# Simple-Robotics/proxsuite

Measured on AMD Instinct MI355X. Metric: QPs/sec (batch, dense backend) at fixed (n, n_eq, n_in); max |KKT residual| vs ref, higher is better.
Workload: dtype f64; 1 GPU; c2: 2048 random dense fp64 QPs per GPU, n=100 n_eq=50 n_in=100, eps_abs=1e-09 eps_rel=0 NO_INITIAL_GUESS (reference generators and seeds, benchmark/timings-parallel.cpp:43-63; BASELINE.json configs); batch_per_gpu=2048, n=100, n_eq=50, n_in=100, threads_per_qp=64, lds_bytes_per_qp=18968, parallelism=batch sharded over 1 GPU(s), dense_backend=PrimalDualLDLT

## Files before the change

### proxsuite_amd/csrc/pqp_capi.hip

```cpp
#include <hip/hip_runtime.h>

#include <algorithm>
#include <cmath>
#include <cstdio>
#include <cstdlib>
#include <cstring>
#include <limits>
#include <string>
#include <vector>

#include "pqp_host.hpp"
#include "pqp_diag.hpp"

namespace {

thread_local std::string g_err;

bool
absent(double v)
{
  return std::isnan(v);
}

int
// ... 254 lines not shown
  const int need = d.nd > d.n ? d.nd : d.n;
  h->nt = need <= 256 ? 256 : (need <= 512 ? 512 : 1024);
  if (need > PQP_MAX_ROWS || pqp::setup_lds_bytes(d, 1024) > 160 * 1024) {
    delete h;
    return fail(PQP_ERR_UNSUPPORTED, "max(n, n_eq + n_in (+ n)) > " + std::to_string(PQP_MAX_ROWS) +
                                       " (or n + n_eq + n_in (+ n) > ~10000) is not supported by this build");
  }
#if PQP_CHUNK_ALL
  if (const char* e = std::getenv("PQP_TEST_NT_MAX")) {
    const int f = std::atoi(e);
    if ((f == 256 || f == 512) && h->nt > f)
      h->nt = f;
  }
#endif
  if (const char* e = std::getenv("PQP_SCHEDULE"))
    h->lpt = std::string(e) == "lpt";
  h->dev.rep_phase = 0;
  h->dev.rep_count = 1;
  h->dev.trace = nullptr;
  h->dev.trace_slot = nullptr;
  h->dev.trace_cap = 0;
  if (const char* e = std::getenv("PQP_REPEAT_PHASE"))
    h->dev.rep_phase = std::atoi(e);
  if (const char* e = std::getenv("PQP_REPEAT_COUNT"))
    h->dev.rep_count = std::atoi(e);
  h->lds_solve = pqp::lds_bytes(d, h->nt);
  h->lds_setup = pqp::setup_lds_bytes(d, h->nt);
  const char* force_hbm = std::getenv("PQP_FORCE_HBM_VECTORS");
  const bool vectors_in_hbm = h->lds_solve > 160 * 1024 || (force_hbm && force_hbm[0] == '1');
  if (vectors_in_hbm)
    h->nt = 1024;
  const size_t B = size_t(batch_size), n = size_t(dim), ne = size_t(n_eq), ni = size_t(n_in),
               nc = size_t(d.nc), nd = size_t(d.nd);
  pqp::Batch& D = h->dev;
  int rc = 0;
#define ALLOC(ptr, cnt)                                                                             \
  if ((rc = dalloc(h, &(ptr), (cnt)))) {                                                            \
    pqp_batch_destroy(h);                                                                           \
    return rc;                                                                                      \
  }                                                                                                 \
  if (B > 0 && size_t(cnt) % B == 0 && (void*)(ptr) != (void*)h->d_order && (void*)(ptr) != (void*)h->d_cmd)           \
    h->per_qp.push_back({ reinterpret_cast<char*>(ptr), (size_t(cnt) / B) * sizeof(*(ptr)) });
  ALLOC(D.H, B * n * n)
  ALLOC(D.g, B * n)
  ALLOC(D.A, B * ne * n)
  ALLOC(D.b, B * ne)
  ALLOC(D.C, B * ni * n)
  ALLOC(D.u, B * ni)
  ALLOC(D.l, B * ni)
  ALLOC(D.u_box, B * n)
  ALLOC(D.l_box, B * n)
  ALLOC(D.Hs, B * n * n)
  ALLOC(D.gs, B * n)
  ALLOC(D.As, B * ne * n)
  ALLOC(D.ATs, B * ne * n)
  ALLOC(D.bs, B * ne)
  ALLOC(D.Cs, B * ni * n)
  ALLOC(D.CTs, B * ni * n)
  ALLOC(D.us, B * ni)
  ALLOC(D.ls, B * ni)
  ALLOC(D.ubs, B * n)
  ALLOC(D.lbs, B * n)
  ALLOC(D.is, B * n)
  ALLOC(D.delta, B * size_t(d.ntot))
  ALLOC(D.x, B * n)
  ALLOC(D.y, B * ne)
  ALLOC(D.z, B * nc)
  ALLOC(D.se, B * ne)
  ALLOC(D.si, B * nc)
  ALLOC(D.info, B)
  ALLOC(D.state, B)
  ALLOC(D.F, B * n * n)
  ALLOC(D.WL, B * n * n)
  ALLOC(D.WU, B * n * n)
  ALLOC(D.dF, B * n)
  ALLOC(D.Zr, B * nd * n)
  ALLOC(D.Zc, B * nd * n)
  ALLOC(D.G, B * nd * nd)
  ALLOC(D.WS, B * nd * nd)
  ALLOC(D.LS, B * nd * nd)
  ALLOC(D.dS, B * nd)
  ALLOC(D.act, B * nc)
  ALLOC(D.stats, B * size_t(pqp::ST_COUNT))
  if (vectors_in_hbm) {
    h->lds_solve = pqp::lds_bytes(d, h->nt);
    h->lds_setup = pqp::setup_lds_bytes(d, h->nt);
    if ((rc = dalloc(h, &h->vec_scratch, B * ((h->lds_solve + 7) / 8)))) {
      pqp_batch_destroy(h);
      return rc;
    }
  }
  ALLOC(h->d_order, B)
  ALLOC(h->d_settings, B)
  ALLOC(h->d_cmd, B)
#undef ALLOC
  D.settings = h->d_settings;
  D.cmd = h->d_cmd;

  h->settings.resize(B);
  for (auto& s : h->settings)
    pqp_settings_default(&s, h->backend);
  h->cmd.assign(B, pqp::Cmd{});
  h->is_initialized.assign(B, 0);
  h->c_diag.assign(B, 0);
  {
    std::vector<pqp_info> info(B);
    for (auto& i : info)
      pqp_info_default(&i, h->backend);
    if (B)
      HIP_TRY(hipMemcpy(D.info, info.data(), B * sizeof(pqp_info), hipMemcpyHostToDevice));
    std::vector<pqp::State> st(B);
    for (auto& s : st) {
      std::memset(&s, 0, sizeof(s));
      s.ruiz_c = 1.0;
    }
    if (B)
      HIP_TRY(hipMemcpy(D.state, st.data(), B * sizeof(pqp::State), hipMemcpyHostToDevice));
    const double ib = std::sqrt(std::numeric_limits<double>::max());
    std::vector<double> tmp;
    auto fill = [&](double* dst, size_t cnt, double v) -> int {
      if (!cnt)
        return PQP_OK;
      tmp.assign(cnt, v);
      HIP_TRY(hipMemcpy(dst, tmp.data(), cnt * sizeof(double), hipMemcpyHostToDevice));
      return PQP_OK;
    };
    if ((rc = fill(D.u, B * ni, +ib)) || (rc = fill(D.l, B * ni, -ib)) ||
        (rc = fill(D.u_box, B * n, +ib)) || (rc = fill(D.l_box, B * n, -ib)) ||
        (rc = fill(D.delta, B * size_t(d.ntot), 1.0)) || (rc = fill(D.is, B * n, 1.0))) {
      pqp_batch_destroy(h);
      return rc;
    }
  }
  HIP_TRY(hipEventCreate(&h->ev0));
  HIP_TRY(hipEventCreate(&h->ev1));
  HIP_TRY(hipEventCreate(&h->ev_mid));
  *out = h;
  return PQP_OK;
}

void
pqp_batch_destroy(pqp_batch* h)
{
  if (!h)
    return;
  (void)settle(h);
  DeviceGuard guard_(h->device);
  for (void* p : h->host_allocs)
    (void)hipHostFree(p);
  if (h->owned_stream)
    (void)hipStreamDestroy(h->owned_stream);
  for (void* p : h->allocs)
    (void)hipFree(p);
  if (h->trace_dev)
    (void)hipFree(h->trace_dev);
  if (h->trace_slot_dev)
    (void)hipFree(h->trace_slot_dev);
  if (h->ev0)
    (void)hipEventDestroy(h->ev0);
  if (h->ev1)
    (void)hipEventDestroy(h->ev1);
  if (h->ev_mid)
    (void)hipEventDestroy(h->ev_mid);
  delete h;
}

// ... 989 lines not shown
```

### proxsuite_amd/csrc/pqp_dwave.hpp

```cpp
#ifndef PQP_DWAVE_HPP
#define PQP_DWAVE_HPP

#include "pqp_diag.hpp"
#include <utility>

namespace pqp {

#ifndef PQP_DW_HB
#define PQP_DW_HB 2
#endif
#ifndef PQP_DW_SCHUR_LAZY
#define PQP_DW_SCHUR_LAZY 1
#endif
#ifndef PQP_DW_SCHUR_REG_BLOCKS
#define PQP_DW_SCHUR_REG_BLOCKS 8
#endif
constexpr int DW_SCHUR_REG_BLOCKS = PQP_DW_SCHUR_REG_BLOCKS;
constexpr int DW_MAXDIM = 128;

enum
{
  DLV_XP = 0,
  DLV_YP,
  DLV_ZP,
// ... 312 lines not shown
      const double qv = (T[0] + T[1]) + (T[2] + T[3]);
      pqp_d4 T2;
#pragma unroll
      for (int k = 0; k < 4; ++k)
        T2[k] = 0.0;
      T2 = mfma_f64_16x16x4(qv, 1.0, T2);
      if (lr == 0) {
#pragma unroll
        for (int k = 0; k < 4; ++k) {
          const int t = g + lk + 4 * k;
          if (t < hi_t)
            rout[t] = T2[k];
        }
      }
    };
    constexpr int HB = (NCB == 1) ? PQP_DW_HB : 1;
    constexpr int GR = (HB >= 2) ? 8 * HB : 16;
    for (int g = lo_t; g < hi_t; g += GR) {
      double p[GR];
#pragma unroll
      for (int h0 = 0; h0 < GR; h0 += 8 * HB) {
        DPair v[HB][8][NCB];
#pragma unroll
        for (int hb = 0; hb < HB; ++hb)
          issue(v[hb], g + h0 + 8 * hb);
        dw_sched_fence();
#pragma unroll
        for (int hb = 0; hb < HB; ++hb)
          consume(v[hb], g + h0 + 8 * hb, p + h0 + 8 * hb);
      }
      if (ROWS) {
#pragma unroll
        for (int k = 0; k < GR; k += 16)
          if (g + k < hi_t)
            reduce16(p + k, g + k);
      }
    }
    if (COLS) {
#pragma unroll
      for (int cb = 0; cb < NCB; ++cb) {
        cacc[cb][0] += acc2[cb][0];
        cacc[cb][1] += acc2[cb][1];
      }
    }
  }
  struct Rows1
  {
    int off[2], nrec[2];
  };
  struct Rows2
  {
    int off[2][2], nrec[2][2];
  };
  __device__ __forceinline__ Rows1 rows_full(int stride, int len, int R) const
  {
    Rows1 w;
    DW_S(s)
    {
      w.off[s] = idx(s) * stride * 8;
      w.nrec[s] = (idx(s) < R) ? w.off[s] + len * 8 : 0;
    }
    return w;
  }
  __device__ __forceinline__ Rows1 rows_tril(int stride, int R) const
  {
    Rows1 w;
    DW_S(s)
    {
      w.off[s] = idx(s) * stride * 8;
      w.nrec[s] = (idx(s) < R) ? w.off[s] + (idx(s) + 1) * 8 : 0;
    }
    return w;
  }
  __device__ __forceinline__ Rows2 rows2_tril(int stride, int R) const
  {
    Rows2 w;
    DW_B(b) DW_S(s)
    {
      w.off[b][s] = didx(b, s) * stride * 8;
      w.nrec[b][s] = (didx(b, s) < R) ? w.off[b][s] + (didx(b, s) + 1) * 8 : 0;
    }
    return w;
  }
  __device__ __forceinline__ Rows1 rows_list(const int (&sel)[2], int stride, int len, int R) const
  {
    Rows1 w;
    DW_S(s)
    {
      w.off[s] = sel[s] * stride * 8;
      w.nrec[s] = (idx(s) < R) ? w.off[s] + len * 8 : 0;
    }
    return w;
  }
  __device__ __forceinline__ Rows2 rows2_list(const int (&sel)[2][2], int stride, int len, int R) const
  {
    Rows2 w;
    DW_B(b) DW_S(s)
    {
      w.off[b][s] = sel[b][s] * stride * 8;
      w.nrec[b][s] = (didx(b, s) < R) ? w.off[b][s] + len * 8 : 0;
    }
    return w;
  }
  template<bool COLS, bool ROWS, int NCB>
  __device__ __forceinline__ void mat_pass2(cgptr base, int t1, const Rows2& w, const double (&cvec)[2][2],
                                            const double (&xop)[NCB][2], double (&cacc)[NCB][2], lptr rout)
  {
    mat_pass_block<COLS, ROWS, NCB, false>(base, 0, t1, w.off[0], w.nrec[0], cvec[0], xop, cacc, rout);
    if (t1 > 128)
      mat_pass_block<COLS, ROWS, NCB, false>(base, 1, t1, w.off[1], w.nrec[1], cvec[1], xop, cacc, rout);
  }
  template<bool COLS, bool ROWS, int NCB, bool LOW = false>
  __device__ __forceinline__ void mat_pass1(cgptr base, int t1, const Rows1& w, const double (&cvec)[2],
                                            const double (&xop)[NCB][2], double (&cacc)[NCB][2], lptr rout)
  {
    mat_pass_block<COLS, ROWS, NCB, LOW>(base, 0, t1, w.off, w.nrec, cvec, xop, cacc, rout);
  }

  __device__ __forceinline__ void hess_mv(const double (&v)[2], double (&out)[2])
  {
    cgptr Hs = P.Hs();
    const int nn = n;
    double dg[2];
    DW_S(s) dg[s] = (idx(s) < nn) ? Hs[(unsigned)(idx(s) * (nn + 1))] : 0.0;
    double acc[1][2] = { { 0.0, 0.0 } };
    const double xop[1][2] = { { v[0], v[1] } };
    mat_pass1<true, true, 1>(Hs, nn, rows_tril(nn, nn), v, xop, acc, scr);
    __syncthreads();
    DW_S(s) out[s] = (idx(s) < nn) ? (acc[0][s] + scr[idx(s)]) - dg[s] * v[s] : 0.0;
    __syncthreads();
  }
  template<bool COLS, bool ROWS>
  __device__ __forceinline__ void dual_pass(cgptr M, int R, const double (&c)[2], const double (&xv)[2], double (&colout)[2],
                                            double (&rowout)[2])
  {
    const int nn = n;
    double acc[1][2] = { { 0.0, 0.0 } };
    const double xop[1][2] = { { xv[0], xv[1] } };
    mat_pass1<COLS, ROWS, 1>(M, R, rows_full(nn, nn, R), c, xop, acc, scr);
    if (COLS) {
      DW_S(s) colout[s] = (idx(s) < nn) ? acc[0][s] : 0.0;
    }
    if (ROWS) {
      __syncthreads();
      DW_S(s) rowout[s] = (idx(s) < R) ? scr[idx(s)] : 0.0;
      __syncthreads();
    }
  }

  __device__ __forceinline__ bool slot_live(int a) const
  {
    const int k = a - ne;
    if (k < 0)
      return true;
    return slot_of[actl[k]] == k;
  }
  __device__ __forceinline__ void zero_dead(double (&v)[2][2]) const
  {
    DW_B(b) DW_S(s)
    {
      const int a = didx(b, s);
      const bool live = (a < r) && slot_live(a < r ? a : 0);
      if (!live)
        v[b][s] = 0.0;
    }
  }
  __device__ __forceinline__ void build_rowid()
  {
    DW_B(b) DW_S(s)
    {
      const int a = didx(b, s);
      if (a < r)
        rowid[a] = (a < ne) ? a : ne + actl[a - ne];
    }
    __syncthreads();
  }

  __device__ __forceinline__ TilePair diag_tile_factor(int k0, int rr, lptr dSl, lptr tile, lptr dinv)
  {
    const int lr = lane & 15, lk = lane >> 4;
    TilePair Pm;
    const int nb = (rr - k0 < 16) ? (rr - k0) : 16;
    const int rw = lane & 15;
    double a[16];
#pragma unroll
    for (int c = 0; c < 16; ++c) {
      const double v = tile[rw * 16 + c];
      a[c] = (rw < nb && c < nb) ? v : ((rw == c) ? 1.0 : 0.0);
    }
#pragma unroll
    for (int c = 0; c < 16; ++c) {
      const double dc = lane_bcast(a[c], c);
      const double l = a[c] / dc;
#pragma unroll
      for (int cp = c + 1; cp < 16; ++cp) {
        const double mcp = lane_bcast(a[c], cp);
        if (rw >= cp)
          a[cp] = fma(-l, mcp, a[cp]);
      }
      if (rw > c)
        a[c] = l;
    }
    __syncthreads();
    if (lane < 16) {
#pragma unroll
      for (int c = 0; c < 16; ++c)
        tile[rw * 16 + c] = (c < rw) ? a[c] : 0.0;
      double dr = 1.0;
#pragma unroll
      for (int c = 0; c < 16; ++c)
// ... 650 lines not shown
    tic();
    bool fadd[2], frm[2];
    DW_S(s)
    {
      const bool want = (fl[s] & 4) != 0, had = (fl[s] & 8) != 0;
      fadd[s] = want && !had;
      frm[s] = !want && had;
    }
    int rka[2], rkr[2], na, nr;
    ranks(fadd, rka, na);
    ranks(frm, rkr, nr);
    if (na + nr == 0 && !schur_dirty) {
      toc(ST_CYC_ZG);
      return;
    }
    const int lim = incr_max(r);
    const bool incremental = !schur_dirty && (na + nr) <= lim && n_slots + na <= ni && (n_slots - n_c) + nr <= lim;
    if (INCR_MAX > 0 && incremental) {
      DW_S(s)
      {
        if (frm[s])
          chg[rkr[s]] = idx(s);
        if (fadd[s])
          chg[INCR_MAX + rka[s]] = idx(s);
      }
      __syncthreads();
      toc(ST_CYC_ZG);
      bool ok = true;
      for (int t = 0; t < nr; ++t) {
        const int i = uni(chg[t]);
        const int sl = uni(slot_of[i]);
        __syncthreads();
        if (lane == 0)
          slot_of[i] = -1;
        DW_S(s) if (idx(s) == i) fl[s] &= ~8;
        __syncthreads();
        schur_delete(sl);
        n_c -= 1;
      }
      for (int t = 0; t < na; ++t) {
        const int i = uni(chg[INCR_MAX + t]);
        ok = schur_append(i) && ok;
        DW_S(s) if (idx(s) == i) fl[s] |= 8;
        n_c += 1;
      }
      schur_incremental = true;
      toc(ST_CYC_SCHUR);
      if (PQP_LIKELY(ok))
        return;
      schur_dirty = true;
      tic();
    }
    bool want[2];
    int rk[2], total;
    DW_S(s) want[s] = (fl[s] & 4) != 0;
    ranks(want, rk, total);
    __syncthreads();
    DW_S(s)
    {
      if (idx(s) < ni) {
        slot_of[idx(s)] = want[s] ? rk[s] : -1;
        if (want[s])
          actl[rk[s]] = idx(s);
      }
      fl[s] = (fl[s] & 7) | (want[s] ? 8 : 0);
    }
    n_c = total;
    n_slots = total;
    r = ne + n_slots;
    schur_dirty = true;
    __syncthreads();
    build_rowid();
    toc(ST_CYC_ZG);
    if (r > 0)
      factor_schur();
    else
      schur_dirty = false;
    toc(ST_CYC_SCHUR);
  }

  __device__ __forceinline__ void kkt_solve_in_place(double (&bx)[2], double (&bd)[2][2])
  {
    const int nn = n, rr = r;
    cgptr WU = P.WU(), WL = P.WL(), Zr = P.Zr();
    double t[2], t2[2];
    {
      double acc[1][2] = { { 0.0, 0.0 } };
      const double xn[1][2] = { { 0.0, 0.0 } };
      mat_pass1<true, false, 1, true>(WU, nn, rows_full(nn, nn, nn), bx, xn, acc, scr);
      DW_S(s)
      {
        t[s] = (idx(s) < nn) ? acc[0][s] : 0.0;
        t2[s] = t[s] / dF[s];
      }
    }
    double t1[2];
    if (rr > 0) {
      int rid[2][2];
      DW_B(b) DW_S(s) rid[b][s] = rowid[didx(b, s)];
      const Rows2 zrows = rows2_list(rid, nn, nn, rr);
      {
        const double xop[1][2] = { { t2[0], t2[1] } };
        double na[1][2] = { { 0.0, 0.0 } };
        double none[2][2] = { { 0.0, 0.0 }, { 0.0, 0.0 } };
        mat_pass2<false, true, 1>(Zr, rr, zrows, none, xop, na, scr);
      }
      __syncthreads();
      DW_B(b) DW_S(s)
      {
        const int a = didx(b, s);
        const bool live = (a < rr) && slot_live(a < rr ? a : 0);
        bd[b][s] = live ? scr[a] - bd[b][s] : 0.0;
      }
      __syncthreads();
      toc(ST_CYC_KKT_SOLVE);
      schur_apply(bd);
      toc(ST_CYC_SOLVE_LDLT);
      double acc[1][2] = { { 0.0, 0.0 } };
      const double xn[1][2] = { { 0.0, 0.0 } };
      mat_pass2<true, false, 1>(Zr, rr, zrows, bd, xn, acc, scr);
      DW_S(s) t1[s] = (idx(s) < nn) ? (t[s] - acc[0][s]) / dF[s] : 0.0;
    } else {
      DW_S(s) t1[s] = t2[s];
    }
    {
      double acc[1][2] = { { 0.0, 0.0 } };
      const double xn[1][2] = { { 0.0, 0.0 } };
      mat_pass1<true, false, 1>(WL, nn, rows_tril(nn, nn), t1, xn, acc, scr);
      DW_S(s) bx[s] = (idx(s) < nn) ? acc[0][s] : 0.0;
    }
    bytes((long)nn * (nn + 1) * 8 + (long)rr * nn * 16);
    count(ST_N_KKT_SOLVES);
  }

  __device__ __forceinline__ double kkt_residual()
  {
    const int nn = n;
    const double rho = info.rho;
    hess_mv(dx, Hdx);
    if (ne > 0) {
      const double c[2] = { sd[0][0], sd[0][1] };
      double cm[2];
      DW_S(s) cm[s] = (idx(s) < ne) ? c[s] : 0.0;
      dual_pass<true, true>(P.As(), ne, cm, dx, ATdy, Adx);
    } else {
      vzero(ATdy);
      vzero(Adx);
    }
    if (ni > 0) {
      __syncthreads();
      to_lds2(scr + 512, sd);
      __syncthreads();
      double zf[2];
      DW_S(s) zf[s] = (idx(s) < ni && active(s)) ? scr[512 + ne + slot_of[idx(s)]] : 0.0;
      __syncthreads();
      dual_pass<true, true>(P.Cs(), ni, zf, dx, CTdz, Cdx);
    } else {
      vzero(CTdz);
      vzero(Cdx);
    }
    double m = 0;
    DW_S(s)
    {
      const double e = (idx(s) < nn) ? rx[s] - rho * dx[s] - Hdx[s] - ATdy[s] - CTdz[s] : 0.0;
      ex[s] = e;
      m = vmax_abs(m, e);
    }
    __syncthreads();
    DW_S(s)
    {
      if (idx(s) < ne)
        scr[idx(s)] = Adx[s];
      if (idx(s) < ni && active(s))
        scr[ne + slot_of[idx(s)]] = Cdx[s];
    }
    __syncthreads();
    DW_B(b) DW_S(s)
    {
      const int a = didx(b, s);
      const bool live = (a < r) && slot_live(a < r ? a : 0);
      double e = 0.0;
      if (live)
        e = (a < ne) ? rd[b][s] - scr[a] + sd[b][s] * info.mu_eq : rd[b][s] - (scr[a] - sd[b][s] * info.mu_in);
      ed[b][s] = e;
      m = vmax_abs(m, e);
    }
    __syncthreads();
    bytes(((long)nn * (nn + 1) / 2 + (long)ne * nn + (long)ni * nn) * 8);
    return lane_max0(m);
  }

  __device__ __forceinline__ bool iterative_solve(double eps)
  {
    vzero(dx);
    dzero(sd);
    vcopy(ex, rx);
    DW_B(b) DW_S(s) ed[b][s] = rd[b][s];
    long it = 0, it_stability = 0;
    UD preverr = 0, cur = 0;
    while (true) {
      tic();
      kkt_solve_in_place(ex, ed);
      DW_S(s) dx[s] += ex[s];
      DW_B(b) DW_S(s) sd[b][s] += ed[b][s];
      toc(ST_CYC_KKT_SOLVE);
      cur = kkt_residual();
      toc(ST_CYC_RESIDUAL);
      ++it;
      if (it > 1) {
        if (cur > preverr)
          it_stability += 1;
// ... 1325 lines not shown
```

### proxsuite_amd/csrc/pqp_solver.hpp

```cpp
#ifndef PQP_SOLVER_HPP
#define PQP_SOLVER_HPP

#include "pqp_block.hpp"
#include "pqp_types.h"

namespace pqp {

#define PQP_UNLIKELY(x) __builtin_expect(!!(x), 0)
#define PQP_LIKELY(x) __builtin_expect(!!(x), 1)

constexpr double MACHINE_EPS = 2.220446049250313e-16;
#ifndef PQP_ZG_DEPTH
#define PQP_ZG_DEPTH 8
#endif
constexpr int ZG_DEPTH = PQP_ZG_DEPTH;
#ifndef PQP_LS_UNROLL
#define PQP_LS_UNROLL 4
#endif
#ifndef PQP_LS_BRACKET
#define PQP_LS_BRACKET 1
#endif
#ifndef PQP_ZG_BLOCK2
#define PQP_ZG_BLOCK2 1
#endif
// ... 82 lines not shown
  int is_initialized;
  int n_c;
  int factor_valid;
  int ls_valid;
  int n_slots;
  int c_diag;
  int ls_edited;
  int scaled_valid;
  int _pad2;
  double ruiz_c;
  double dual_feasibility_rhs_2;
  double correction_guess_rhs_g;
  double mu_eq_fact, mu_in_fact, rho_fact;
};

enum
{
  ST_CYC_TOTAL = 0,
  ST_CYC_SCALE,
  ST_CYC_FACTOR_H,
  ST_CYC_ZG,
  ST_CYC_SCHUR,
  ST_CYC_KKT_SOLVE,
  ST_CYC_RESIDUAL,
  ST_CYC_LINESEARCH,
  ST_CYC_GLOBAL_RES,
  ST_CYC_NEWTON_MISC,
  ST_N_NEWTON,
  ST_N_SCHUR_FACT,
  ST_N_NEW_ROWS,
  ST_N_KKT_SOLVES,
  ST_N_LS_BREAKPOINTS,
  ST_N_ACTIVE_FINAL,
  ST_CYC_F_LOAD,
  ST_CYC_F_UPDATE,
  ST_CYC_F_PANEL,
  ST_CYC_F_WRITEBACK,
  ST_CYC_F_TINV,
  ST_CYC_S_GATHER,
  ST_CYC_SOLVE_LDLT,
  ST_N_SCHUR_BLOCKED,
  ST_N_APPEND,
  ST_N_DELETE,
  ST_BYTES_ENGINE,
  ST_N_REFACTORIZE,
  ST_CYC_LS_EVAL,
  ST_CYC_CERT,
  ST_CYC_UPDATE,
  ST_WALL_TICKS,
  ST_FLOPS_FACT,
  ST_COUNT
};

struct Batch
{
  Dims d;
  long B;
  double *H, *g, *A, *b, *C, *u, *l, *u_box, *l_box;
  double *Hs, *gs, *As, *ATs, *bs, *Cs, *CTs, *us, *ls, *ubs, *lbs, *is;
  double* delta;
  double *x, *y, *z, *se, *si;
  pqp_info* info;
  const pqp_settings* settings;
  State* state;
  const Cmd* cmd;
  double *F;
  double *WL, *WU;
  double *dF;
  double *Zr;
  double *Zc;
  double *G;
  double *WS;
  double *LS;
  double *dS;
  int* act;
  long long* stats;
  double wall_us_per_tick;
  int rep_phase, rep_count;
  double *hx, *hy, *hz, *hse, *hsi;
  pqp_info* hinfo;
  double* trace;
  const int* trace_slot;
  int trace_cap;
};

struct BackwardArgs
{
  const double* ld;
  double eps, rho_new, mu_new;
  double *dL_dH, *dL_dg, *dL_dA, *dL_db, *dL_dC, *dL_du, *dL_dl;
  long first;
  const int* order;
};

#ifndef PQP_VECTORS_IN_HBM
#define PQP_VECTORS_IN_HBM 0
#endif
#define ZG_LDS_TILED(nt) ((nt) >= 512 && !PQP_VECTORS_IN_HBM)
template<int NT>
struct Lds
{
  static constexpr int SH = ZG_LDS_TILED(NT) ? 2 : 0;
  static constexpr int DF = ZG_LDS_TILED(NT) ? 0 : 14;
  lptr base;
  int n, ne, nc, ni, nd, tmax, nt, plen;
  int o_ne, o_nc, o_ni, o_nd, o_t2;
  __device__ __forceinline__ lptr at(int off) const
  {
    PQP_OPAQUE_VECTOR(off);
    return base + off;
  }
#define PQP_LVEC(name, cls_off, len, slot) \
  __device__ __forceinline__ lptr name() const { return at((cls_off) + (slot) * (len)); }
  PQP_LVEC(dF, 0, n, DF)
  PQP_LVEC(t1, 0, n, DF + 1)
  PQP_LVEC(x, 0, n, SH + 0)
  PQP_LVEC(xp, 0, n, SH + 1)
  PQP_LVEC(gs, 0, n, SH + 2)
  PQP_LVEC(ubs, 0, n, SH + 3)
  PQP_LVEC(lbs, 0, n, SH + 4)
  PQP_LVEC(isc, 0, n, SH + 5)
  PQP_LVEC(dx, 0, n, SH + 6)
  PQP_LVEC(rx, 0, n, SH + 7)
  PQP_LVEC(ex, 0, n, SH + 8)
  PQP_LVEC(Hdx, 0, n, SH + 9)
  PQP_LVEC(ATdy, 0, n, SH + 10)
  PQP_LVEC(CTdz, 0, n, SH + 11)
  PQP_LVEC(CTzin, 0, n, SH + 12)
  PQP_LVEC(dres, 0, n, SH + 13)
  PQP_LVEC(y, o_ne, ne, 0)
  PQP_LVEC(yp, o_ne, ne, 1)
  PQP_LVEC(bs, o_ne, ne, 2)
  PQP_LVEC(dy, o_ne, ne, 3)
  PQP_LVEC(Adx, o_ne, ne, 4)
  PQP_LVEC(se, o_ne, ne, 5)
  PQP_LVEC(z, o_nc, nc, 0)
  PQP_LVEC(zp, o_nc, nc, 1)
  PQP_LVEC(dz, o_nc, nc, 2)
  PQP_LVEC(Cdx, o_nc, nc, 3)
  PQP_LVEC(si, o_nc, nc, 4)
  PQP_LVEC(rup, o_nc, nc, 5)
  PQP_LVEC(zfull, o_nc, nc, 6)
  PQP_LVEC(us, o_ni, ni, 0)
  PQP_LVEC(ls, o_ni, ni, 1)
  PQP_LVEC(rd, o_nd, nd, 0)
  PQP_LVEC(ed, o_nd, nd, 1)
  PQP_LVEC(sd, o_nd, nd, 2)
  PQP_LVEC(dS, o_nd, nd, 3)
#undef PQP_LVEC
  __device__ __forceinline__ lptr stage() const { return at(2 * n); }
  __device__ __forceinline__ int part_len() const { return plen; }
  __device__ __forceinline__ int red_len() const { return 2 * RED_VALS * (nt / WAVE) + 8; }
  __device__ __forceinline__ lptr t2() const { return at(o_t2); }
  __device__ __forceinline__ lptr part() const { return at(o_t2 + tmax); }
  __device__ __forceinline__ lptr red() const { return at(o_t2 + tmax + part_len()); }
  __device__ __forceinline__ lptr top() const { return at(o_t2 + tmax + part_len() + red_len()); }
  __device__ __forceinline__ PQP_LDS long long* stat() const
  {
    return (PQP_LDS long long*)at(o_t2 + tmax + part_len() + red_len() + TOP_DOUBLES + PARK_DOUBLES);
  }
  __device__ __forceinline__ lptr park() const { return at(o_t2 + tmax + part_len() + red_len() + TOP_DOUBLES); }
  __device__ __forceinline__ liptr ints(int off) const
  {
    liptr q = (liptr)(base + (o_t2 + tmax + part_len() + red_len() + TOP_DOUBLES + PARK_DOUBLES + ST_COUNT + 1));
    PQP_OPAQUE_VECTOR(off);
    return q + off;
  }
// ... 50 lines not shown
{
  size_t ints = (size_t)d.nc * 3 + d.nd + nt / WAVE + 16 + 2 * INCR_MAX;
  return lds_doubles(d, nt) * sizeof(double) + ints * sizeof(int) + 64;
}

template<int NT>
__device__ __forceinline__ void
lds_carve(Lds<NT>& L, lptr base, const Dims& d, int nt)
{
  L.base = base;
  L.n = uni(d.n);
  L.ne = uni(d.n_eq);
  L.nc = uni(d.nc);
  L.ni = uni(d.n_in);
  L.nd = uni(d.nd);
  L.tmax = uni(d.nd > d.n ? d.nd : d.n);
  L.nt = nt;
  L.plen = uni(lds_part_len(d.n, d.n_eq, d.nc, d.n_in, d.nd, nt));
  L.o_ne = uni(16 * L.n);
  L.o_nc = uni(L.o_ne + 6 * L.ne);
  L.o_ni = uni(L.o_nc + 7 * L.nc);
  L.o_nd = uni(L.o_ni + 2 * L.ni);
  L.o_t2 = uni(L.o_nd + 4 * L.nd);
}

struct QpRef
{
  const Batch& b;
  const long q;
  __device__ __forceinline__ QpRef(const Batch& b_, long q_)
    : b(b_)
    , q(q_)
  {
  }
  __device__ __forceinline__ long n() const { return b.d.n; }
  __device__ __forceinline__ long ne() const { return b.d.n_eq; }
  __device__ __forceinline__ long ni() const { return b.d.n_in; }
  __device__ __forceinline__ long nc() const { return b.d.nc; }
  __device__ __forceinline__ long nd() const { return b.d.nd; }
  __device__ __forceinline__ long lq() const
  {
    long v = q;
    PQP_OPAQUE_SCALAR(v);
    return v;
  }
#define PQP_PTR(name, stride) \
  __device__ __forceinline__ gptr name() const { return (gptr)(b.name + lq() * (stride)); }
  PQP_PTR(H, n() * n())
  PQP_PTR(g, n())
  PQP_PTR(A, ne() * n())
  PQP_PTR(C, ni() * n())
  PQP_PTR(u, ni())
  PQP_PTR(l, ni())
  PQP_PTR(u_box, n())
  PQP_PTR(l_box, n())
  PQP_PTR(Hs, n() * n())
  PQP_PTR(gs, n())
  PQP_PTR(As, ne() * n())
  PQP_PTR(ATs, ne() * n())
  PQP_PTR(bs, ne())
  PQP_PTR(Cs, ni() * n())
  PQP_PTR(CTs, ni() * n())
  PQP_PTR(us, ni())
  PQP_PTR(ls, ni())
  PQP_PTR(ubs, n())
  PQP_PTR(lbs, n())
  PQP_PTR(is, n())
  PQP_PTR(delta, (long)b.d.ntot)
  PQP_PTR(x, n())
  PQP_PTR(y, ne())
  PQP_PTR(z, nc())
  PQP_PTR(se, ne())
  PQP_PTR(si, nc())
  PQP_PTR(F, n() * n())
  PQP_PTR(WL, n() * n())
  PQP_PTR(WU, n() * n())
  PQP_PTR(dF, n())
  PQP_PTR(Zr, nd() * n())
  PQP_PTR(Zc, nd() * n())
  PQP_PTR(G, nd() * nd())
  PQP_PTR(WS, nd() * nd())
  PQP_PTR(LS, nd() * nd())
  PQP_PTR(dS, nd())
#undef PQP_PTR
  __device__ __forceinline__ gptr bvec() const { return (gptr)(b.b + q * ne()); }
  __device__ __forceinline__ PQP_GLOBAL int* act() const { return (PQP_GLOBAL int*)(b.act + q * nc()); }
  __device__ __forceinline__ PQP_GLOBAL long long* stats() const
  {
    return (PQP_GLOBAL long long*)(b.stats + q * ST_COUNT);
  }
  __device__ __forceinline__ pqp_info* info() const { return b.info + q; }
  __device__ __forceinline__ State* state() const { return b.state + q; }
  __device__ __forceinline__ const pqp_settings& settings() const { return b.settings[q]; }
  __device__ __forceinline__ cgptr dlt_x() const { return delta(); }
  __device__ __forceinline__ cgptr dlt_eq() const { return delta() + n(); }
  __device__ __forceinline__ cgptr dlt_in() const { return delta() + n() + ne(); }
  __device__ __forceinline__ cgptr dlt_box() const { return delta() + n() + ne() + ni(); }
};

__device__ __forceinline__ bool
absent(double v)
{
  return v != v;
}

struct UInfo
{
  UD mu_eq, mu_eq_inv, mu_in, mu_in_inv, rho, nu;
  long iter, iter_ext, mu_updates, rho_updates;
  UD setup_time, solve_time, run_time, objValue, pri_res, dua_res, duality_gap, iterative_residual,
    minimal_H_eigenvalue_estimate;
  int status;
  __device__ __forceinline__ void load(const pqp_info& o)
  {
    mu_eq = o.mu_eq;
    mu_eq_inv = o.mu_eq_inv;
    mu_in = o.mu_in;
    mu_in_inv = o.mu_in_inv;
    rho = o.rho;
    nu = o.nu;
    iter = uni((long)o.iter);
    iter_ext = uni((long)o.iter_ext);
    mu_updates = uni((long)o.mu_updates);
    rho_updates = uni((long)o.rho_updates);
    setup_time = o.setup_time;
    solve_time = o.solve_time;
    run_time = o.run_time;
    objValue = o.objValue;
    pri_res = o.pri_res;
    dua_res = o.dua_res;
    duality_gap = o.duality_gap;
    iterative_residual = o.iterative_residual;
    minimal_H_eigenvalue_estimate = o.minimal_H_eigenvalue_estimate;
    status = uni((int)o.status);
  }
  __device__ __forceinline__ void store(pqp_info& o) const
  {
    o.mu_eq = mu_eq;
    o.mu_eq_inv = mu_eq_inv;
    o.mu_in = mu_in;
    o.mu_in_inv = mu_in_inv;
    o.rho = rho;
    o.nu = nu;
    o.iter = iter;
    o.iter_ext = iter_ext;
    o.mu_updates = mu_updates;
    o.rho_updates = rho_updates;
    o.setup_time = setup_time;
    o.solve_time = solve_time;
    o.run_time = run_time;
    o.objValue = objValue;
    o.pri_res = pri_res;
    o.dua_res = dua_res;
    o.duality_gap = duality_gap;
    o.iterative_residual = iterative_residual;
    o.minimal_H_eigenvalue_estimate = minimal_H_eigenvalue_estimate;
    o.status = status;
    o._pad = 0;
  }
};

template<typename Info>
__device__ __forceinline__ void
cleanup_statistics(Info& i)
{
  i.run_time = 0;
// ... 3631 lines not shown
    vstore(P.se(), L.se(), ne);
    vstore(P.si(), L.si(), nc);
    vstore(P.dS(), L.dS(), d.nd);
    if (batch.hx) {
      vstore((gptr)(batch.hx + P.lq() * n), L.x(), n);
      vstore((gptr)(batch.hy + P.lq() * ne), L.y(), ne);
      vstore((gptr)(batch.hz + P.lq() * nc), L.z(), nc);
      vstore((gptr)(batch.hse + P.lq() * ne), L.se(), ne);
      vstore((gptr)(batch.hsi + P.lq() * nc), L.si(), nc);
    }
    if (pm())
      vstore(P.dF(), L.dF(), n);
    {
      PQP_GLOBAL int* ga = P.act();
      for (int i = threadIdx.x; i < nc; i += NT)
        ga[i] = act_pack((i < n_slots && slot_live(ne + i)) ? L.act()[i] : -1, L.aflags()[i]);
    }
    __syncthreads();
    if (threadIdx.x == 0) {
      L.stat()[ST_WALL_TICKS] += wall_clock64();
      if (st.compute_timings) {
        info.solve_time = (double)L.stat()[ST_WALL_TICKS] * batch.wall_us_per_tick;
        info.run_time = info.solve_time + info.setup_time;
      }
      info.store(*P.info());
      if (batch.hinfo)
        info.store(batch.hinfo[q]);
      W.dirty = 1;
      W.is_initialized = 1;
      W.n_c = n_c;
      W.n_slots = n_slots;
      W.factor_valid = 1;
      W.ls_valid = schur_dirty ? 0 : 1;
      W.ls_edited = schur_incremental ? 1 : 0;
      W.mu_eq_fact = info.mu_eq;
      W.mu_in_fact = info.mu_in;
      W.rho_fact = info.rho;
      *P.state() = W;
      L.stat()[ST_N_ACTIVE_FINAL] = n_c;
      L.stat()[ST_CYC_TOTAL] += clock64();
      PQP_GLOBAL long long* gs = P.stats();
      for (int k = 0; k < ST_COUNT; ++k)
        gs[k] = L.stat()[k];
    }
  }

  __device__ __forceinline__ void prologue()
  {
    const int ne = d.n_eq;
    const State W = *P.state();
    set_diag_mode(W);
    info.load(*P.info());
    ruiz_c = W.ruiz_c;
#ifdef PQP_STATS
    for (int k = threadIdx.x; k < ST_COUNT; k += NT)
      L.stat()[k] = 0;
    __syncthreads();
#endif
    const int ig = st.initial_guess;
    const bool wswpr = (ig == PQP_WARM_START_WITH_PREVIOUS_RESULT);
    const bool dirty = W.dirty != 0;
    const bool do_rescale = dirty && !wswpr;
    bool do_factor = true;
    if (dirty && !wswpr)
      cold_start(info, st);
    if (wswpr && !((!dirty && W.refactorize) || !W.factor_valid))
      do_factor = false;
    if (do_rescale) {
      tic();
      lptr S = L.rd();
      vload(S, P.delta(), d.ntot);
      __syncthreads();
      const bool rewrite_matrices = W.scaled_valid == 0;
      write_scaled<NT>(batch, q, S, ruiz_c, false, dm(), rewrite_matrices);
      if (rewrite_matrices)
        bytes(((long)d.n * d.n * 2 + 3L * ne * d.n + 3L * d.n_in * d.n) * 8);
      toc(ST_CYC_SCALE);
    }
    if (do_factor) {
      tic();
      factor_primal_block();
      toc(ST_CYC_FACTOR_H);
    }
#ifdef PQP_STATS
    __syncthreads();
    if (threadIdx.x == 0) {
      PQP_GLOBAL long long* gs = P.stats();
      for (int k = 0; k < ST_COUNT; ++k)
        gs[k] = L.stat()[k];
    }
#endif
  }

  __device__ __forceinline__ void backward(const BackwardArgs& bw, long slot_in_launch)
  {
    const int n = d.n, ne = d.n_eq, ni = d.n_in;
    const long ntot = (long)n + ne + ni;
    cgptr ld = (cgptr)(bw.ld + slot_in_launch * ntot);
    for (int k = threadIdx.x; k < ST_COUNT; k += NT)
      L.stat()[k] = 0;
    {
      const State& Wr = *P.state();
      diag_mode = (SPEC == 0) && d.hessian != PQP_HESSIAN_DENSE && d.n_eq == 0 && Wr.c_diag != 0 &&
                  !(d.n_in > 0 && d.box != 0);
      ruiz_c = Wr.ruiz_c;
    }
    info.load(*P.info());
    const double c = ruiz_c;
    vload(L.x(), P.x(), n);
    vload(L.y(), P.y(), ne);
    vload(L.z(), P.z(), ni);
    cgptr dX = P.dlt_x(), dE = P.dlt_eq(), dI = P.dlt_in();
    for (int k = threadIdx.x; k < n; k += NT)
      L.dx()[k] = P.x()[k] / dX[k];
    for (int i = threadIdx.x; i < ni; i += NT) {
      L.aflags()[i] = 0;
      L.slot_of()[i] = -1;
    }
    __syncthreads();
    if (ni > 0) {
      if (dm()) {
        cgptr cd = P.CTs();
        for (int i = threadIdx.x; i < ni; i += NT)
          L.Cdx()[i] = cd[i] * L.dx()[i];
        __syncthreads();
      } else {
        mv(P.CTs(), ni, n, ni, L.dx(), L.Cdx());
      }
      cgptr gu = P.u(), gl = P.l();
      for (int i = threadIdx.x; i < ni; i += NT) {
        const double ctz = L.Cdx()[i] / dI[i] + L.z()[i];
        const bool up = (ctz - gu[i]) >= 0., lo = (ctz - gl[i]) <= 0.;
        L.aflags()[i] = (up ? 1 : 0) | (lo ? 2 : 0) | ((up || lo) ? 4 : 0);
      }
      __syncthreads();
    }
    info.rho = bw.rho_new;
    info.mu_eq = bw.mu_new;
    info.mu_in = bw.mu_new;
    factor_primal_block<false>();
    n_c = 0;
    n_slots = 0;
    r = ne;
    schur_dirty = true;
    apply_active_set();
    const int na = n_c;
    for (int k = threadIdx.x; k < n; k += NT)
      L.rx()[k] = -ld[k] * (dX[k] * c);
    for (int k = threadIdx.x; k < ne; k += NT)
      L.rd()[k] = -ld[n + k] * dE[k];
    double in_any = 0.0;
    for (int i = threadIdx.x; i < ni; i += NT)
      in_any = fmax(in_any, fabs(ld[n + ne + i]));
    in_any = R.max(in_any);
    for (int i = threadIdx.x; i < ni; i += NT) {
      const int a = L.slot_of()[i];
      if (a >= 0) {
        double v = 0.0;
        if (in_any != 0.0) {
          v = -ld[n + ne + i];
          const double s = dI[a];
          for (int t = i; t < ni; ++t)
            v *= s;
        }
        L.rd()[ne + a] = v;
      }
    }
    __syncthreads();
    (void)iterative_solve(bw.eps);
    for (int k = threadIdx.x; k < n; k += NT)
      L.ex()[k] = L.dx()[k] * dX[k];
    for (int k = threadIdx.x; k < ne; k += NT)
      L.ed()[k] = L.sd()[k] * dE[k] / c;
    for (int j = threadIdx.x; j < ni; j += NT) {
// ... 76 lines not shown
```

Before: 272,300 QPs/s.

## Store triangular factors and Hessian in packed global layout for solves

Adds packed lower/upper triangular copies of WL, WU and the Hessian, built once after factorization by a new pack_triangles pass. The Hessian matvec and KKT triangular passes then read these packed buffers instead of full n×n matrices, with new row-offset helpers. The aim is to cut global memory traffic and cache footprint in the solve path, which runs many times per QP. In exchange it adds extra allocations and a packing pass after every setup or refactorization, and the layout uses pair-row granularity for even-aligned access.

```diff
diff --git a/proxsuite_amd/csrc/pqp_capi.hip b/proxsuite_amd/csrc/pqp_capi.hip
--- a/proxsuite_amd/csrc/pqp_capi.hip
+++ b/proxsuite_amd/csrc/pqp_capi.hip
@@ -360,6 +360,9 @@
   ALLOC(D.dS, B * nd)
   ALLOC(D.act, B * nc)
   ALLOC(D.stats, B * size_t(pqp::ST_COUNT))
+  ALLOC(D.WLp, B * size_t(pqp::tril_packed_size(long(n))))
+  ALLOC(D.WUp, B * size_t(pqp::triu_packed_size(long(n))))
+  ALLOC(D.Hsp, B * size_t(pqp::tril_packed_size(long(n))))
   if (vectors_in_hbm) {
     h->lds_solve = pqp::lds_bytes(d, h->nt);
     h->lds_setup = pqp::setup_lds_bytes(d, h->nt);
diff --git a/proxsuite_amd/csrc/pqp_dwave.hpp b/proxsuite_amd/csrc/pqp_dwave.hpp
--- a/proxsuite_amd/csrc/pqp_dwave.hpp
+++ b/proxsuite_amd/csrc/pqp_dwave.hpp
@@ -418,6 +418,26 @@
     }
     return w;
   }
+  __device__ __forceinline__ Rows1 rows_tril_packed(int R) const
+  {
+    Rows1 w;
+    DW_S(s)
+    {
+      w.off[s] = (int)tril_packed_off(idx(s)) * 8;
+      w.nrec[s] = (idx(s) < R) ? w.off[s] + (idx(s) + 1) * 8 : 0;
+    }
+    return w;
+  }
+  __device__ __forceinline__ Rows1 rows_triu_packed(int nn) const
+  {
+    Rows1 w;
+    DW_S(s)
+    {
+      w.off[s] = ((int)triu_packed_off(idx(s), nn) - (idx(s) & ~1)) * 8;
+      w.nrec[s] = (idx(s) < nn) ? w.off[s] + nn * 8 : 0;
+    }
+    return w;
+  }
   __device__ __forceinline__ Rows1 rows_list(const int (&sel)[2], int stride, int len, int R) const
   {
     Rows1 w;
@@ -455,13 +475,13 @@
 
   __device__ __forceinline__ void hess_mv(const double (&v)[2], double (&out)[2])
   {
-    cgptr Hs = P.Hs();
+    cgptr Hs = P.Hsp();
     const int nn = n;
     double dg[2];
-    DW_S(s) dg[s] = (idx(s) < nn) ? Hs[(unsigned)(idx(s) * (nn + 1))] : 0.0;
+    DW_S(s) dg[s] = (idx(s) < nn) ? Hs[(unsigned)(tril_packed_off(idx(s)) + idx(s))] : 0.0;
     double acc[1][2] = { { 0.0, 0.0 } };
     const double xop[1][2] = { { v[0], v[1] } };
-    mat_pass1<true, true, 1>(Hs, nn, rows_tril(nn, nn), v, xop, acc, scr);
+    mat_pass1<true, true, 1>(Hs, nn, rows_tril_packed(nn), v, xop, acc, scr);
     __syncthreads();
     DW_S(s) out[s] = (idx(s) < nn) ? (acc[0][s] + scr[idx(s)]) - dg[s] * v[s] : 0.0;
     __syncthreads();
@@ -1278,12 +1298,12 @@
   __device__ __forceinline__ void kkt_solve_in_place(double (&bx)[2], double (&bd)[2][2])
   {
     const int nn = n, rr = r;
-    cgptr WU = P.WU(), WL = P.WL(), Zr = P.Zr();
+    cgptr WU = P.WUp(), WL = P.WLp(), Zr = P.Zr();
     double t[2], t2[2];
     {
       double acc[1][2] = { { 0.0, 0.0 } };
       const double xn[1][2] = { { 0.0, 0.0 } };
-      mat_pass1<true, false, 1, true>(WU, nn, rows_full(nn, nn, nn), bx, xn, acc, scr);
+      mat_pass1<true, false, 1, true>(WU, nn, rows_triu_packed(nn), bx, xn, acc, scr);
       DW_S(s)
       {
         t[s] = (idx(s) < nn) ? acc[0][s] : 0.0;
@@ -1322,7 +1342,7 @@
     {
       double acc[1][2] = { { 0.0, 0.0 } };
       const double xn[1][2] = { { 0.0, 0.0 } };
-      mat_pass1<true, false, 1>(WL, nn, rows_tril(nn, nn), t1, xn, acc, scr);
+      mat_pass1<true, false, 1>(WL, nn, rows_tril_packed(nn), t1, xn, acc, scr);
       DW_S(s) bx[s] = (idx(s) < nn) ? acc[0][s] : 0.0;
     }
     bytes((long)nn * (nn + 1) * 8 + (long)rr * nn * 16);
diff --git a/proxsuite_amd/csrc/pqp_solver.hpp b/proxsuite_amd/csrc/pqp_solver.hpp
--- a/proxsuite_amd/csrc/pqp_solver.hpp
+++ b/proxsuite_amd/csrc/pqp_solver.hpp
@@ -188,7 +188,31 @@
   double* trace;
   const int* trace_slot;
   int trace_cap;
+  double *WLp, *WUp;
+  double* Hsp;
 };
+
+__host__ __device__ inline long
+tril_packed_off(long t)
+{
+  return 2 * ((t >> 1) + 1) * ((t + 1) >> 1);
+}
+__host__ __device__ inline long
+triu_packed_off(long k, long n)
+{
+  const long e = (n + 1) & ~1L, m = k >> 1;
+  return 2 * m * (e - m + 1) + ((k & 1) ? e - 2 * m : 0);
+}
+__host__ __device__ inline long
+tril_packed_size(long n)
+{
+  return (tril_packed_off(n) + 15) & ~15L;
+}
+__host__ __device__ inline long
+triu_packed_size(long n)
+{
+  return (triu_packed_off(n, n) + 15) & ~15L;
+}
 
 struct BackwardArgs
 {
@@ -405,6 +429,9 @@
   PQP_PTR(WS, nd() * nd())
   PQP_PTR(LS, nd() * nd())
   PQP_PTR(dS, nd())
+  PQP_PTR(WLp, tril_packed_size(n()))
+  PQP_PTR(WUp, triu_packed_size(n()))
+  PQP_PTR(Hsp, tril_packed_size(n()))
 #undef PQP_PTR
   __device__ __forceinline__ gptr bvec() const { return (gptr)(b.b + q * ne()); }
   __device__ __forceinline__ PQP_GLOBAL int* act() const { return (PQP_GLOBAL int*)(b.act + q * nc()); }
@@ -4202,6 +4229,7 @@
       factor_primal_block();
       toc(ST_CYC_FACTOR_H);
     }
+    pack_triangles();
 #ifdef PQP_STATS
     __syncthreads();
     if (threadIdx.x == 0) {
@@ -4210,6 +4238,42 @@
         gs[k] = L.stat()[k];
     }
 #endif
+  }
+
+  __device__ __forceinline__ void pack_triangles()
+  {
+    constexpr int U = 8;
+    const int nn = d.n, tot = nn * nn;
+    cgptr WL = P.WL(), WU = P.WU(), Hs = P.Hs();
+    gptr WLp = P.WLp(), WUp = P.WUp(), Hsp = P.Hsp();
+    __syncthreads();
+    for (int i0 = threadIdx.x; i0 < tot; i0 += U * NT) {
+      double l[U], h[U], u[U];
+      int t[U], c[U];
+#pragma unroll
+      for (int k = 0; k < U; ++k) {
+        const int i = i0 + k * NT;
+        t[k] = i / nn;
+        c[k] = i - t[k] * nn;
+        const bool low = i < tot && c[k] <= t[k], up = i < tot && c[k] >= (t[k] & ~1);
+        l[k] = low ? WL[i] : 0.0;
+        h[k] = low ? Hs[i] : 0.0;
+        u[k] = up ? WU[i] : 0.0;
+      }
+#pragma unroll
+      for (int k = 0; k < U; ++k) {
+        const int i = i0 + k * NT;
+        if (i < tot && c[k] <= t[k]) {
+          const int o = (int)tril_packed_off(t[k]) + c[k];
+          WLp[o] = l[k];
+          Hsp[o] = h[k];
+        }
+        if (i < tot && c[k] >= (t[k] & ~1))
+          WUp[(int)triu_packed_off(t[k], nn) - (t[k] & ~1) + c[k]] = u[k];
+      }
+    }
+    const long used = (long)nn * (nn + 1) + (triu_packed_off(nn, nn) - (long)(nn & 1) * nn);
+    bytes(2 * used * 8);
   }
 
   __device__ __forceinline__ void backward(const BackwardArgs& bw, long slot_in_launch)
```

Result: faster. 278,500 QPs/s (median of 6 runs) (+2.3%).
